# AIGC-Audio/AudioGPT

Hardware: AMD Instinct MI355X
Metric: generated audio-seconds/sec (10s clip, 100 DDIM steps) [3 independent batches of 8 prompts in flight per GPU] (higher is better)
Workload: dtype bf16x3; 1 GPU; Make-An-Audio T2A batch=8/GPU, 100 DDIM steps, CFG 1.5, UNet+VAE+HiFi-GAN(16k), fp32 storage, bf16x3-split MFMA (hi/lo, fp32 accumulate; meets the fp32 parity gates); prompts_per_gpu=8, ddim_steps=100, mel_frames=624, hipgraph=True, batches_in_flight=3, cfg_lanes=1, concurrency_hint=3, parallelism=prompt-sharded x1 (RCCL bcast cond / gather wav)

## Files before the change

### audiogpt_amd/_lib.py

```python
import ctypes as C
import os

import torch

_HERE = os.path.dirname(os.path.abspath(__file__))
LIB_PATH = os.environ.get("AUDIOGPT_AMD_LIB") or os.path.join(_HERE, "libaudiogpt_mi355x.so")


class MaaError(RuntimeError):
    pass


class maa_tensor(C.Structure):
    _fields_ = [("name", C.c_char_p), ("data", C.POINTER(C.c_float)), ("ndim", C.c_int), ("shape", C.c_int64 * 6)]


class maa_prof_row(C.Structure):
    _fields_ = [("name", C.c_char * 48), ("launches", C.c_int64), ("ms", C.c_double), ("flops", C.c_double),
                ("bytes", C.c_double)]


class maa_unet_config(C.Structure):
    _fields_ = [("in_channels", C.c_int), ("out_channels", C.c_int), ("model_channels", C.c_int),
                ("num_res_blocks", C.c_int),
# ... 114 lines not shown
    sig = {
        "maa_ctx_create": [ci, vp, C.POINTER(vp)],
        "maa_ctx_destroy": [vp],
        "maa_ctx_synchronize": [vp],
        "maa_ctx_set_stream": [vp, vp],
        "maa_ctx_workspace_bytes": [vp, C.POINTER(C.c_size_t)],
        "maa_ctx_set_precision": [vp, ci],
        "maa_ctx_set_cfg_split": [vp, ci],
        "maa_ctx_set_concurrency": [vp, ci],
        "maa_ctx_reload_tuning": [vp],
        "maa_prof_begin": [vp, ci],
        "maa_prof_end": [vp, C.POINTER(maa_prof_row), ci, C.POINTER(ci)],
        "maa_unet_create": [vp, C.POINTER(maa_unet_config), C.POINTER(maa_tensor), ci, C.POINTER(vp)],
        "maa_unet_destroy": [vp],
        "maa_unet_set_context": [vp, vp, vp, ci, ci],
        "maa_unet_forward": [vp, vp, vp, vp, ci, ci, ci, vp],
        "maa_ddim_update": [vp, vp, vp, vp, cf, vp, C.c_int64, vp, vp],
        "maa_ddim_sample": [vp, vp, C.POINTER(maa_ddim_args), vp],
        "maa_ddim_stochastic_encode": [vp, vp, ci, cf, vp, vp, fp, fp, ci, vp, ci, ci, ci, ci, vp],
        "maa_ddim_decode": [vp, vp, C.POINTER(maa_ddim_args), ci, vp],
        "maa_ldm_plms_sample": [vp, vp, C.POINTER(maa_ddim_args), vp],
        "maa_ddpm_sample": [vp, vp, C.POINTER(maa_ddpm_args), vp],
        "maa_ddpm_update": [vp, vp, vp, vp, fp, fp, fp, fp, fp, ci, vp, cf, ci, ci, ci, ci, ci, vp, vp],
        "maa_vae_create": [vp, C.POINTER(maa_vae_config), C.POINTER(maa_tensor), ci, C.POINTER(vp)],
        "maa_vae_destroy": [vp],
        "maa_vae_decode": [vp, vp, vp, ci, ci, ci, cf, vp],
        "maa_vae_decode_spec": [vp, vp, vp, ci, ci, ci, cf, vp],
        "maa_vae_encode_moments": [vp, vp, vp, ci, ci, ci, vp],
        "maa_vocoder_create": [vp, C.POINTER(maa_vocoder_config), C.POINTER(maa_tensor), ci, C.POINTER(vp)],
        "maa_vocoder_destroy": [vp],
        "maa_vocoder_forward": [vp, vp, vp, ci, ci, vp],
        "maa_vocoder_forward_f0": [vp, vp, vp, vp, vp, vp, ci, ci, vp],
        "maa_diffnet_create": [vp, C.POINTER(maa_diffnet_config), C.POINTER(maa_tensor), ci, C.POINTER(vp)],
        "maa_diffnet_destroy": [vp],
        "maa_diffnet_forward": [vp, vp, vp, vp, vp, ci, ci, vp],
        "maa_plms_sample": [vp, vp, C.POINTER(maa_plms_args), vp],
        "maa_ds_ddpm_sample": [vp, vp, C.POINTER(maa_ds_ddpm_args), vp],
        "maa_ds_ddpm_update": [vp, vp, vp, vp, fp, fp, fp, fp, fp, ci, ci, ci, ci, ci, vp],
        "maa_encoder_create": [vp, C.POINTER(maa_encoder_config), C.POINTER(maa_tensor), ci, C.POINTER(vp)],
        "maa_encoder_destroy": [vp],
        "maa_encoder_text": [vp, vp, vp, ci, ci, vp],
        "maa_encoder_image": [vp, vp, vp, ci, vp],
        "maa_encoder_text_cls": [vp, vp, vp, ci, ci, vp],
        "maa_clap_audio_create": [vp, C.POINTER(maa_clap_audio_config), C.POINTER(maa_tensor), ci, C.POINTER(vp)],
        "maa_clap_audio_destroy": [vp],
        "maa_clap_audio_embed": [vp, vp, vp, ci, ci, vp, vp],
        "maa_clap_similarity": [vp, vp, vp, ci, ci, ci, cf, vp],
        "maa_spectral_create": [vp, C.POINTER(maa_spectral_config), fp, fp, C.POINTER(vp)],
        "maa_spectral_destroy": [vp],
        "maa_spectral_forward": [vp, vp, vp, ci, ci, vp],
        "maa_resampler_create": [vp, ci, ci, ci, ci, fp, C.POINTER(vp)],
        "maa_resampler_destroy": [vp],
        "maa_resampler_forward": [vp, vp, vp, ci, ci, vp],
        "maa_op_linear": [vp, vp, ci, ci, fp, fp, ci, ci, vp],
        "maa_op_conv": [vp, vp, ci, ci, ci, ci, fp, fp, ci, ci, ci, ci, ci, ci, ci, cf, vp, ci, ci],
        "maa_op_groupnorm": [vp, vp, ci, ci, ci, fp, fp, cf, ci, vp],
        "maa_op_layernorm": [vp, vp, ci, ci, fp, fp, cf, vp],
        "maa_op_attention": [vp, vp, vp, vp, ci, ci, ci, ci, ci, cf, vp],
        "maa_op_attention_ex": [vp, vp, ci, ci, vp, ci, ci, vp, ci, ci, ci, ci, ci, ci, ci, cf, vp, ci, ci, ci],
        "maa_op_conv_transpose1d": [vp, vp, ci, ci, ci, fp, fp, ci, ci, ci, cf, vp],
        "maa_op_snake_aa": [vp, vp, ci, ci, ci, fp, fp, ci, vp],
        "maa_op_bench_conv": [vp, ci, ci, ci, ci, ci, ci, ci, ci, C.POINTER(C.c_float)],
        "maa_calib": [vp, ci, C.POINTER(C.c_double)],
        "maa_op_mrf_pair": [vp, vp, ci, ci, ci, fp, fp, ci, ci, cf, fp, fp, ci, ci, cf, cf, ci, vp],
        "maa_op_groupnorm_ex": [vp, vp, ci, ci, vp, ci, ci, ci, ci, ci, fp, fp, cf, ci, vp, ci, vp],
        "maa_op_layernorm_ex": [vp, vp, ci, ci, fp, fp, cf, vp, ci],
        "maa_op_split32": [vp, vp, ci, ci, cf, ci, vp],
        "maa_unet_forward_split": [vp, vp, vp, vp, vp, ci, ci, ci, ci, ci, ci, ci, fp, vp],
        "maa_op_unfold": [vp, vp, ci, ci, ci, ci, ci, ci, ci, ci, vp],
        "maa_op_fold": [vp, vp, fp, ci, ci, ci, ci, ci, ci, ci, ci, vp],
    }
    for name, argtypes in sig.items():
        fn = getattr(lib, name)
        fn.argtypes = argtypes
        fn.restype = ci
    _lib = lib
    return lib


def check(status):
    if status != 0:
        raise MaaError("libaudiogpt_mi355x: %s (status %d)" % (load().maa_last_error().decode(), status))


def host_f32(t):
    t = t.detach().to(device="cpu", dtype=torch.float32).contiguous()
    return t, C.cast(t.data_ptr(), C.POINTER(C.c_float))


def tensor_list(state_dict):
    items = list(state_dict.items())
    arr = (maa_tensor * len(items))()
    keep = []
    for i, (name, t) in enumerate(items):
        ht, ptr = host_f32(t)
        bname = name.encode()
        keep.append((ht, bname))
        arr[i].name = bname
        arr[i].data = ptr
        arr[i].ndim = ht.dim()
        for d, s in enumerate(ht.shape):
            arr[i].shape[d] = s
    return arr, len(items), keep


def dptr(t):
    assert t.is_cuda and t.dtype == torch.float32 and t.is_contiguous(), (t.device, t.dtype, t.is_contiguous())
    return C.c_void_p(t.data_ptr())
# ... 1 lines not shown
```

### audiogpt_amd/backend.py

```python
import ctypes as C
import threading
import weakref

import numpy as np
import torch

from . import _lib as L


def default_precision():
    import os
    p = os.environ.get("AUDIOGPT_AMD_PRECISION", "bf16x3")
    if p not in Context.PRECISIONS:
        raise ValueError("AUDIOGPT_AMD_PRECISION must be one of %s" % sorted(Context.PRECISIONS))
    return p


_contexts = weakref.WeakSet()


def reload_tuning():
    for c in list(_contexts):
        c.reload_tuning()

# ... 26 lines not shown

    def reload_tuning(self):
        if getattr(self, "h", None):
            with self.lock:
                L.check(self.lib.maa_ctx_reload_tuning(self.h))

    def set_precision(self, precision):
        L.check(self.lib.maa_ctx_set_precision(self.h, self.PRECISIONS[precision]))
        self.precision = precision

    def set_cfg_split(self, mode):
        L.check(self.lib.maa_ctx_set_cfg_split(self.h, -1 if mode is None else int(bool(mode))))

    def set_concurrency(self, n):
        L.check(self.lib.maa_ctx_set_concurrency(self.h, -1 if n is None else int(n)))

    def synchronize(self):
        L.check(self.lib.maa_ctx_synchronize(self.h))

    def workspace_bytes(self):
        n = C.c_size_t()
        L.check(self.lib.maa_ctx_workspace_bytes(self.h, C.byref(n)))
        return n.value

    def prof_begin(self, detail=False):
        L.check(self.lib.maa_prof_begin(self.h, int(detail)))

    def prof_end(self):
        rows = (L.maa_prof_row * 512)()
        n = C.c_int()
        L.check(self.lib.maa_prof_end(self.h, rows, 512, C.byref(n)))
        return {rows[i].name.decode(): dict(launches=int(rows[i].launches), ms=rows[i].ms, flops=rows[i].flops,
                                            bytes=rows[i].bytes) for i in range(n.value)}

    def calib(self):
        out = {}
        for kind, key in ((0, "mfma_bf16_tflops"), (1, "copy_gbs"), (2, "l2_read_gbs"), (3, "infinity_cache_read_gbs")):
            v = C.c_double()
            L.check(self.lib.maa_calib(self.h, kind, C.byref(v)))
            out[key] = v.value
        return out

    def close(self):
        if getattr(self, "h", None):
            self.lib.maa_ctx_destroy(self.h)
            self.h = None

    def __del__(self):
        try:
            self.close()
        except Exception:
            pass

    def op_linear(self, a, w, b=None, geglu=False):
        a = _f32(a, self.device)
        M, K = a.shape
        N = w.shape[0]
        wt, wp = L.host_f32(w)
        bt, bp = L.host_f32(b) if b is not None else (None, None)
        y = torch.empty(M, N // 2 if geglu else N, device=self.device)
        L.check(self.lib.maa_op_linear(self.h, L.dptr(a), M, K, wp, bp, N, int(geglu), L.dptr(y)))
        return y

    def op_conv(self, x, w, b=None, stride=1, pad=0, dil=1, up=False, leaky=0.0, out_hw=None):
        x = _f32(x, self.device)
        B, Cin, H, W = x.shape
        Cout, _, KH, KW = w.shape
        if out_hw is None:
            He, We = (2 * H, 2 * W) if up else (H, W)
            ph = pad if KH > 1 else 0
            Ho = (He + 2 * ph - dil * (KH - 1) - 1) // stride + 1
            Wo = (We + 2 * pad - dil * (KW - 1) - 1) // stride + 1
        else:
            Ho, Wo = out_hw
        wt, wp = L.host_f32(w)
        bt, bp = L.host_f32(b) if b is not None else (None, None)
        y = torch.empty(B, Cout, Ho, Wo, device=self.device)
        L.check(self.lib.maa_op_conv(self.h, L.dptr(x), B, Cin, H, W, wp, bp, Cout, KH, KW, stride, pad, dil,
                                     int(up), float(leaky), L.dptr(y), Ho, Wo))
        return y

    def op_groupnorm(self, x, gamma, beta, eps, silu=False):
        x = _f32(x, self.device)
        B, Cc = x.shape[:2]
        HW = int(np.prod(x.shape[2:]))
        gt, gp = L.host_f32(gamma)
        bt, bp = L.host_f32(beta)
        y = torch.empty_like(x)
        L.check(self.lib.maa_op_groupnorm(self.h, L.dptr(x), B, Cc, HW, gp, bp, float(eps), int(silu), L.dptr(y)))
        return y

    def op_layernorm(self, x, gamma, beta, eps=1e-5):
        x = _f32(x, self.device)
        rows, Cc = x.reshape(-1, x.shape[-1]).shape
        gt, gp = L.host_f32(gamma)
        bt, bp = L.host_f32(beta)
        y = torch.empty_like(x)
        L.check(self.lib.maa_op_layernorm(self.h, L.dptr(x), rows, Cc, gp, bp, float(eps), L.dptr(y)))
        return y

    def op_attention(self, q, k, v, heads, alpha):
        q, k, v = _f32(q, self.device), _f32(k, self.device), _f32(v, self.device)
        B, Nq, Cc = q.shape
        Nk = k.shape[1]
        y = torch.empty_like(q)
        L.check(self.lib.maa_op_attention(self.h, L.dptr(q), L.dptr(k), L.dptr(v), B, heads, Cc // heads, Nq, Nk,
                                          float(alpha), L.dptr(y)))
        return y

    def op_attention_ex(self, q, ldq, hsq, k, ldk, hsk, v, ldv, hsv, B, heads, dh, Nq, Nk, alpha, out, ldo,
                        out_split=0, causal=0):
        for t in (q, k, v, out):
            assert t.is_cuda and t.dtype == torch.float32, (t.device, t.dtype)
        L.check(self.lib.maa_op_attention_ex(self.h, C.c_void_p(q.data_ptr()), int(ldq), int(hsq),
                                             C.c_void_p(k.data_ptr()), int(ldk), int(hsk),
                                             C.c_void_p(v.data_ptr()), int(ldv), int(hsv), int(B), int(heads), int(dh),
                                             int(Nq), int(Nk), float(alpha), C.c_void_p(out.data_ptr()), int(ldo),
                                             int(out_split), int(causal)))
        return out

    def op_groupnorm_ex(self, x1, ld1, C1, x2, ld2, C2, B, HW, groups, gamma, beta, eps, silu, out, out_split=0, raw=None):
        for t in (x1, x2, out, raw):
            assert t is None or (t.is_cuda and t.dtype == torch.float32), (t.device, t.dtype)
        gt, gp = L.host_f32(gamma)
        bt, bp = L.host_f32(beta)
        assert gt.numel() == C1 + C2 and bt.numel() == C1 + C2
        ptr = lambda t: C.c_void_p(t.data_ptr()) if t is not None else None
        L.check(self.lib.maa_op_groupnorm_ex(self.h, ptr(x1), int(ld1), int(C1), ptr(x2), int(ld2), int(C2), int(B), int(HW),
                                             int(groups), gp, bp, float(eps), int(silu), ptr(out), int(out_split), ptr(raw)))
        return out

    def op_layernorm_ex(self, x, gamma, beta, eps=1e-5, out_split=0):
# ... 951 lines not shown
```

### audiogpt_amd/csrc/api.cpp

```cpp
#include "models.h"

#include <cstdint>
#include <cstring>
#include <memory>

namespace maa {
const char* last_error_cstr();
}

struct maa_ctx {
    maa::Ctx c;
    bool owns_stream = false;
};
struct maa_unet {
    std::unique_ptr<maa::UNet> m;
};
struct maa_vae {
    std::unique_ptr<maa::VAE> m;
};
struct maa_vocoder {
    std::unique_ptr<maa::Vocoder> m;
};
struct maa_diffnet {
    std::unique_ptr<maa::DiffNet> m;
// ... 556 lines not shown
}

int maa_spectral_create(maa_ctx* ctx, const maa_spectral_config* cfg, const float* h_basis, const float* h_melw,
                        maa_spectral** out) {
    return guarded([&] {
        bind(ctx);
        MAA_CHECK(cfg && h_basis && h_melw && out, "bad spectral arguments");
        MAA_CHECK(cfg->n_fft > 0 && cfg->n_fft % 4 == 0 && cfg->hop > 0 && cfg->hop % 4 == 0 && cfg->n_freq == cfg->n_fft / 2 + 1 &&
                      cfg->n_mels > 0 && (cfg->pad_mode == 0 || cfg->pad_mode == 1) && (cfg->power == 1 || cfg->power == 2) &&
                      (cfg->log_kind == 0 || cfg->log_kind == 1) && cfg->amin > 0.f && (cfg->out_layout == 0 || cfg->out_layout == 1),
                  "bad spectral config (n_fft and hop must be multiples of 4)");
        auto* s = new maa_spectral;
        s->m.reset(new maa::Spectral(*cfg, h_basis, h_melw));
        *out = s;
    });
}
int maa_spectral_destroy(maa_spectral* s) {
    return guarded([&] { delete s; });
}
int maa_spectral_forward(maa_ctx* ctx, maa_spectral* s, const float* d_wav, int B, int n, float* d_out) {
    return guarded([&] {
        bind(ctx);
        MAA_CHECK(s && d_wav && d_out && B > 0 && n > 0, "bad spectral_forward arguments");
        MAA_CHECK(s->m->config().pad_mode == 0 || n > s->m->config().n_fft / 2, "signal too short for reflect padding");
        s->m->forward(ctx->c, d_wav, B, n, d_out);
    });
}

int maa_resampler_create(maa_ctx* ctx, int orig, int neu, int width, int klen, const float* h_kernels, maa_resampler** out) {
    return guarded([&] {
        bind(ctx);
        MAA_CHECK(out && h_kernels && orig > 0 && neu > 0 && width > 0 && klen > 0, "bad resampler arguments");
        auto* r = new maa_resampler;
        r->m.reset(new maa::Resampler(orig, neu, width, klen, h_kernels));
        *out = r;
    });
}
int maa_resampler_destroy(maa_resampler* r) {
    return guarded([&] { delete r; });
}
int maa_resampler_forward(maa_ctx* ctx, maa_resampler* r, const float* d_wav, int B, int n, float* d_out) {
    return guarded([&] {
        bind(ctx);
        MAA_CHECK(r && d_wav && d_out && B > 0 && n > 0, "bad resampler_forward arguments");
        r->m->forward(ctx->c, d_wav, B, n, d_out);
    });
}

static bool op_presplit(const maa::Ctx& c, int channels, bool other_prologue) {
    return c.tune.op_presplit && c.dtype != 0 && channels % 32 == 0 && !other_prologue;
}

int maa_op_linear(maa_ctx* ctx, const float* d_a, int M, int K, const float* h_w, const float* h_bias, int N,
                  int geglu, float* d_y) {
    return guarded([&] {
        bind(ctx);
        MAA_CHECK(d_a && h_w && d_y && M > 0 && K > 0 && N > 0, "bad op_linear arguments");
        OneShot s;
        s.add("w", h_w, {N, K});
        if (h_bias) s.add("b", h_bias, {N});
        maa::WeightStore ws(ctx->c.dtype != 0);
        maa::Ctx& c = ctx->c;
        MAA_CHECK(!geglu || h_bias, "geglu needs a bias");
        maa::PackedW pw = geglu ? ws.pack_geglu(s.sd, "w", "b") : ws.pack_conv(s.sd, "w", h_bias ? "b" : "", 1, 1);
        const bool pre = op_presplit(c, K, false);
        maa::run_sized(c, [&] {
            const float* a = d_a;
            if (pre) {
                float* sp = c.ws.alloc_f((size_t)M * K);
                maa::launch_split32_pack(c, d_a, M, K, sp);
                a = sp;
            }
            maa::linear_into(c, a, K, M, K, pw, nullptr, 0, d_y, geglu ? N / 2 : N, geglu, 0, pre ? M : 0);
        });
        MAA_HIP(hipStreamSynchronize(c.stream));
    });
}

int maa_op_conv(maa_ctx* ctx, const float* d_x, int B, int Cin, int H, int W, const float* h_w, const float* h_bias,
                int Cout, int KH, int KW, int stride, int pad, int dil, int upsample2, float leaky_slope, float* d_y,
                int Ho, int Wo) {
    return guarded([&] {
        bind(ctx);
        MAA_CHECK(d_x && h_w && d_y, "bad op_conv arguments");
        OneShot s;
        s.add("w", h_w, {Cout, Cin, KH, KW});
        if (h_bias) s.add("b", h_bias, {Cout});
        maa::WeightStore ws(ctx->c.dtype != 0);
        maa::Ctx& c = ctx->c;
        maa::PackedW pw = ws.pack_conv(s.sd, "w", h_bias ? "b" : "", KH, KW);
        maa::PackedW pw4;
        if (upsample2 && KH == 3 && KW == 3 && stride == 1 && pad == 1 && dil == 1 && leaky_slope == 0.f)
            pw4 = ws.pack_conv_up2(s.sd, "w", h_bias ? "b" : "");
        maa::run_sized(c, [&] {
            maa::T4 x = maa::alloc_t(c, B, H, W, Cin);
            maa::launch_nchw_to_nhwc(c, d_x, B, Cin, H * W, x.p);
            if (!pw4.w && op_presplit(c, Cin, leaky_slope != 0.f)) {
                maa::T4 xs = maa::alloc_t(c, B, H, W, Cin);
                maa::launch_split32_pack(c, x.p, (long long)B * H * W, Cin, xs.p);
                xs.split = true;
                x = xs;
            }
            if (x.split && Cout <= 4 && h_bias && KH == 3 && KW == 3 && stride == 1 && pad == 1 && dil == 1 && !upsample2 && c.tune.up2) {
                maa::PackedW pn = ws.pack_narrow3x3(s.sd, "w", "b");
                if (maa::launch_narrow_conv3x3(c, x.p, Cin, B, H, W, Cin, pn.w, pn.bias, Cout, d_y)) return;
            }
            maa::T4 y = maa::alloc_t(c, B, Ho, Wo, Cout);
            maa::ConvOpt o;
            o.KH = KH;
            o.KW = KW;
            o.stride = stride;
            o.pad = pad;
            o.dil = dil;
            o.up = upsample2;
            if (leaky_slope != 0.f) {
                o.a_act = 1;
                o.a_slope = leaky_slope;
            }
            if (!(pw4.w && maa::conv_up2_into(c, x, pw4, y))) maa::conv_into(c, x, nullptr, pw, o, y);
            maa::launch_nhwc_to_nchw(c, y.p, B, Cout, Ho * Wo, d_y, Cout);
        });
        MAA_HIP(hipStreamSynchronize(c.stream));
    });
}

int maa_calib(maa_ctx* ctx, int kind, double* out_value) {
    return guarded([&] {
        bind(ctx);
        MAA_CHECK(out_value && kind >= 0 && kind <= 3, "bad calib arguments");
        *out_value = maa::calib_run(ctx->c, kind);
    });
}

int maa_op_groupnorm(maa_ctx* ctx, const float* d_x, int B, int C, int HW, const float* h_gamma, const float* h_beta,
                     float eps, int silu, float* d_y) {
    return guarded([&] {
        bind(ctx);
        MAA_CHECK(d_x && h_gamma && h_beta && d_y, "bad op_groupnorm arguments");
        maa::WeightStore ws(ctx->c.dtype != 0);
        maa::Ctx& c = ctx->c;
        float* g = ws.upload(std::vector<float>(h_gamma, h_gamma + C));
        float* b = ws.upload(std::vector<float>(h_beta, h_beta + C));
        maa::run_sized(c, [&] {
            maa::T4 x = maa::alloc_t(c, B, 1, HW, C), y = maa::alloc_t(c, B, 1, HW, C);
            maa::launch_nchw_to_nhwc(c, d_x, B, C, HW, x.p);
            maa::launch_groupnorm(c, x.p, C, C, nullptr, 0, 0, B, HW, 32, g, b, eps, silu, y.p);
            maa::launch_nhwc_to_nchw(c, y.p, B, C, HW, d_y, C);
        });
        MAA_HIP(hipStreamSynchronize(c.stream));
    });
}

int maa_op_layernorm(maa_ctx* ctx, const float* d_x, int rows, int C, const float* h_gamma, const float* h_beta,
                     float eps, float* d_y) {
    return guarded([&] {
        bind(ctx);
        MAA_CHECK(d_x && h_gamma && h_beta && d_y, "bad op_layernorm arguments");
        maa::WeightStore ws(ctx->c.dtype != 0);
        maa::Ctx& c = ctx->c;
        float* g = ws.upload(std::vector<float>(h_gamma, h_gamma + C));
        float* b = ws.upload(std::vector<float>(h_beta, h_beta + C));
        maa::launch_layernorm(c, d_x, rows, C, g, b, eps, d_y);
        MAA_HIP(hipStreamSynchronize(c.stream));
    });
}

int maa_op_attention(maa_ctx* ctx, const float* d_q, const float* d_k, const float* d_v, int B, int heads, int dh,
                     int Nq, int Nk, float alpha, float* d_y) {
    return guarded([&] {
        bind(ctx);
// ... 312 lines not shown
```

### audiogpt_amd/csrc/igemm_dma2.hip

```cpp
#include "igemm_epilogue.h"

#include <cstdio>
#include <cstdlib>
#include <cstring>
#include <type_traits>

namespace maa {

namespace {

template <int BM, int BN, int WGM, int WGN, int NS, int TERMS>
__global__ __launch_bounds__(64 * WGM * WGN) void igemm_dma2_kernel(const IGemm p, int ntiles, int tiles, int Nb,
                                                                     int cps, int items, float* __restrict__ part) {
    constexpr int NW = WGM * WGN, NTH = 64 * NW;
    constexpr int WTM = BM / WGM, WTN = BN / WGN;
    constexpr int MI = WTM / 32, NI = WTN / 32;
    constexpr int ROWS = BM + BN;
    constexpr int STAGE = ROWS * 128;
    constexpr int AI = BM / 8 / NW, BI = BN / 8 / NW;
    constexpr int IPW = AI + BI;
    static_assert(BM % (8 * NW) == 0 && BN % (8 * NW) == 0 && NW % 2 == 0, "copy assignment");
    static_assert(WTM % 32 == 0 && WTN % 32 == 0 && BM % 32 == 0, "tile");
    static_assert(NS >= 3 && (NS - 2) * IPW <= 63, "stages / vmcnt field");
    extern __shared__ __attribute__((aligned(1024))) char smem[];
// ... 187 lines not shown
        zero_acc();
        c_w += w_step;
        if (c_w >= w_cnt) return false;
        c_rem = item_chunks(c_w);
        return true;
    };

    setup_item(g_w);
    c_rem = item_chunks(c_w);
#pragma unroll
    for (int s = 0; s < NS - 1; ++s) issue(s);

    {
        wait_vmcnt<(NS - 2) * IPW>();
        __builtin_amdgcn_s_barrier();
        Frags f0, f1;
        read_frags(smem, 0, f0);
        int st = 0;
        for (;;) {
            const char* cur = smem + st * STAGE;
            const int st_next = st + 1 == NS ? 0 : st + 1;
            const int st_fill = st == 0 ? NS - 1 : st - 1;
            read_frags(cur, 1, f1);
            __builtin_amdgcn_sched_barrier(0);
            mma(f0);
            __builtin_amdgcn_sched_barrier(0);
            wait_vmcnt<(NS - 3) * IPW>();
            __builtin_amdgcn_s_barrier();
            read_frags(smem + st_next * STAGE, 0, f0);
            __builtin_amdgcn_sched_barrier(0);
            static_for<0, TERMS * MI * NI>([&](auto xc) {
                constexpr int x = decltype(xc)::value;
                constexpr int t = x / (MI * NI) + (3 - TERMS), i = (x % (MI * NI)) / NI, j = x % NI;
                if constexpr (t == 0)
                    acc[i][j] = __builtin_amdgcn_mfma_f32_32x32x16_bf16(f1.al[i], f1.bh[j], acc[i][j], 0, 0, 0);
                else if constexpr (t == 1)
                    acc[i][j] = __builtin_amdgcn_mfma_f32_32x32x16_bf16(f1.ah[i], f1.bl[j], acc[i][j], 0, 0, 0);
                else
                    acc[i][j] = __builtin_amdgcn_mfma_f32_32x32x16_bf16(f1.ah[i], f1.bh[j], acc[i][j], 0, 0, 0);
                if constexpr (x < IPW) copy1(st_fill, xc);
                __builtin_amdgcn_sched_barrier(0);
            });
            if constexpr (IPW > TERMS * MI * NI)
                static_for<TERMS * MI * NI, IPW>([&](auto jc) { copy1(st_fill, jc); });
            advance();
            st = st_next;
            if (--c_rem == 0)
                if (!finish_item()) break;
        }
    }
    wait_vmcnt<0>();
}

template <int JW>
__global__ void splitk_reduce_kernel(const IGemm p, const float* __restrict__ part, int S, int tiles, int ntiles, int Nb,
                                     int BM, int BN, int WGN, int MI, int NI) {
    const int NTH = blockDim.x;
    const int tid = threadIdx.x, lane = tid & 63, wid = tid >> 6;
    const int njb = NI / JW, nblk = MI * njb;
    const int wi = xcd_contiguous((int)blockIdx.x, (int)gridDim.x);
    const int tile = wi / nblk, blk = wi - tile * nblk;
    const int i = blk / njb, j = (blk - i * njb) * JW;
    const int mt = tile / ntiles, nt = tile - mt * ntiles;
    const int wm = wid / WGN, wn = wid - wm * WGN;
    const int WTM = 32 * MI, WTN = 32 * NI;
    f32x16 acc[1][JW];
    const long long slab = (long long)(MI * NI * 4) * NTH * 4;
#pragma unroll
    for (int jj = 0; jj < JW; ++jj) {
        const float* src = part + (long long)tile * slab + ((long long)((i * NI + j + jj) * 4) * NTH + tid) * 4;
        f32x4 v[4];
#pragma unroll
        for (int q = 0; q < 4; ++q) v[q] = *reinterpret_cast<const f32x4*>(src + (long long)q * NTH * 4);
        for (int s = 1; s < S; ++s) {
            const float* sp = src + (long long)s * tiles * slab;
#pragma unroll
            for (int q = 0; q < 4; ++q) v[q] += *reinterpret_cast<const f32x4*>(sp + (long long)q * NTH * 4);
        }
#pragma unroll
        for (int q = 0; q < 4; ++q)
#pragma unroll
            for (int e = 0; e < 4; ++e) acc[0][jj][4 * q + e] = v[q][e];
    }
    const int rpb = p.Hout * p.Wout;
    igemm_epilogue<1, JW>(p, acc, mt * BM + wm * WTM + i * 32, nt * BN + wn * WTN + j * 32, lane & 31, lane >> 5, 0, Nb, rpb);
}

template <int BM, int BN, int WGM, int WGN, int NS>
void launch_one(const Ctx& ctx, const IGemm& p, int Nb, int S, float* part) {
    constexpr int NW = WGM * WGN, NTH = 64 * NW;
    constexpr int MI = BM / WGM / 32, NI = BN / WGN / 32;
    const int ncols = p.N * (p.geglu ? 2 : 1);
    const int mtiles = (p.M + BM - 1) / BM, ntiles = (ncols + BN - 1) / BN;
    const int tiles = mtiles * ntiles;
    const int nchunks = p.K / BK;
    const int cps = (nchunks + S - 1) / S;
    const int Seff = (nchunks + cps - 1) / cps;
    MAA_CHECK(Seff == S, "split-K plan leaves an empty slice");
    MAA_CHECK(!p.geglu || NI % 2 == 0, "GEGLU needs value / gate block pairs inside a wave");
    constexpr size_t lds = (size_t)NS * (BM + BN) * 128;
    static_assert(lds <= 163840, "LDS per workgroup");
    const long long items = (long long)tiles * S;
    long long grid = items;
    {
        const int per_cu = (int)(163840 / lds) < 32 / NW ? (int)(163840 / lds) : 32 / NW;
        const long long cap = (long long)device_cu_count(ctx.device) * (per_cu < 1 ? 1 : per_cu);
        if (grid > cap) grid = cap;
    }
    auto go = [&](auto kern) {
        ensure_dynamic_lds(reinterpret_cast<const void*>(kern), ctx.device, (int)lds);
        hipLaunchKernelGGL(kern, dim3((unsigned)grid), dim3(NTH), lds, ctx.stream, p, ntiles, tiles, Nb, cps, (int)items,
                           S > 1 ? part : nullptr);
    };
    if (ctx.dtype == 2)
        go(igemm_dma2_kernel<BM, BN, WGM, WGN, NS, 1>);
    else
        go(igemm_dma2_kernel<BM, BN, WGM, WGN, NS, 3>);
    if (S > 1) launch_splitk_reduce(ctx, p, part, S, tiles, ntiles, Nb, BM, BN, WGN, MI, NI, NTH);
}

}

void launch_splitk_reduce(const Ctx& ctx, const IGemm& p, const float* part, int S, int tiles, int ntiles, int Nb, int BM,
                          int BN, int WGN, int MI, int NI, int NTH) {
    if (p.geglu && NI % 2 == 0) {
        hipLaunchKernelGGL(splitk_reduce_kernel<2>, dim3((unsigned)(tiles * MI * (NI / 2))), dim3(NTH), 0, ctx.stream, p, part, S,
                           tiles, ntiles, Nb, BM, BN, WGN, MI, NI);
        return;
    }
    MAA_CHECK(!p.geglu, "split-K reduce: GEGLU needs value / gate block pairs inside a wave");
    hipLaunchKernelGGL(splitk_reduce_kernel<1>, dim3((unsigned)(tiles * MI * NI)), dim3(NTH), 0, ctx.stream, p, part, S, tiles,
                       ntiles, Nb, BM, BN, WGN, MI, NI);
}

bool igemm_dma2_takes(const Ctx& ctx, const IGemm& p, IGemmPlan& pl) {
    const int ncols = p.N * (p.geglu ? 2 : 1);
    int S = 0;
    if (!ctx.tune.dma2.empty()) {
        if (ctx.tune.dma2 == "off") return false;
        int cfg = 0, ns = 4, pipe = 1, s = 1, kmin = 0, kmax = 1 << 30;
        const int k = std::sscanf(ctx.tune.dma2.c_str(), "%d,%d,%d,%d,%d,%d", &cfg, &ns, &pipe, &s, &kmin, &kmax);
        if (k >= 4) {
            if (p.K < kmin) return false;
            if (p.K <= kmax) S = s < 1 ? 1 : s;
        }
    }
    if (S == 0) {
        if (p.K < 2048 || ncols < 128 || p.geglu) return false;
        S = 2;
    }
    pl.engine = IGemmPlan::DMA2;
    pl.cfg = 0;
    pl.S = fit_slices(p.K / BK, S);
    return true;
}

void launch_igemm_dma2(const Ctx& ctx, const IGemm& p, const IGemmPlan& pl, float* part) {
    MAA_CHECK(pl.S == 1 || part != nullptr, "igemm_dma2: split-K needs its slab workspace");
    launch_one<128, 128, 2, 2, 4>(ctx, p, pl.Nb, pl.S, part);
}

}
```

### audiogpt_amd/csrc/igemm_epilogue.h

```cpp
#pragma once
#include "igemm_device.h"
#include "maa_internal.h"

namespace maa {

__device__ __forceinline__ float fast_erff(float x) {
    const float t = fminf(fabsf(x), 4.0f);
    const float s = t * t;
    float r = -5.654105860e-04f;
    r = fmaf(r, s, 4.923277665e-03f);
    r = fmaf(r, s, -2.671638510e-02f);
    r = fmaf(r, s, 1.128036441e-01f);
    r = fmaf(r, s, -3.761234978e-01f);
    r = fmaf(r, s, 1.128379127e+00f);
    const float small = r * t;
    float q = 1.330939039e-05f;
    q = fmaf(q, t, -3.175720346e-04f);
    q = fmaf(q, t, 3.436867598e-03f);
    q = fmaf(q, t, -2.262198592e-02f);
    q = fmaf(q, t, 1.033189800e-01f);
    q = fmaf(q, t, 6.390933195e-01f);
    q = fmaf(q, t, 1.125925949e+00f);
    q = fmaf(q, t, 7.569686250e-04f);
    const float large = 1.0f - __builtin_amdgcn_exp2f(q * -1.4426950408889634f);
    return copysignf(t < 1.0f ? small : large, x);
}

__device__ __forceinline__ void settle(float& x) { asm volatile("" : "+v"(x)); }

__device__ __forceinline__ void store_split_pair(float* row, int n, float v) {
    const __bf16 h = (__bf16)v;
    const unsigned hb = __builtin_bit_cast(unsigned short, h);
    const __bf16 l = (__bf16)(v - __builtin_bit_cast(float, hb << 16));
    const unsigned lb = __builtin_bit_cast(unsigned short, l);
    const bool even = (n & 1) == 0;
    const unsigned mine = even ? lb : hb;
    const unsigned theirs = (unsigned)__builtin_amdgcn_update_dpp(0, (int)mine, 0xB1, 0xF, 0xF, false);
    unsigned* o = reinterpret_cast<unsigned*>(reinterpret_cast<unsigned short*>(row) + (n >> 5) * 64 + ((n & 31) & ~1) + (even ? 0 : 32));
    *o = even ? (hb | (theirs << 16)) : (theirs | (lb << 16));
}

template <int MI, int NI, bool PAIR>
__device__ __forceinline__ void igemm_epilogue_impl(const IGemm& p, f32x16 (&acc)[MI][NI], int m_base, int n_base,
                                                    int lrow, int lk, long long coff, int Nb, int rpb) {
    float* cp = p.c + coff;
    const float* resp = p.res ? p.res + coff : nullptr;
    if (p.geglu) {
        if constexpr (NI % 2 == 0) {
#pragma unroll
            for (int i = 0; i < MI; ++i)
#pragma unroll
                for (int j = 0; j < NI; j += 2) {
                    const int cpk = n_base + j * 32 + lrow;
                    const int ncol = (cpk >> 6) * 32 + lrow;
                    if (cpk + 32 < Nb && ncol < p.N) {
                        float bv = p.bias ? p.bias[cpk] : 0.f;
                        float bg = p.bias ? p.bias[cpk + 32] : 0.f;
                        settle(bv);
                        settle(bg);
                        float outv[16];
#pragma unroll
                        for (int r = 0; r < 16; ++r) {
                            const float val = acc[i][j][r] * p.alpha + bv;
                            const float g = acc[i][j + 1][r] * p.alpha + bg;
                            const float gl = 0.5f * g * (1.f + fast_erff(g * 0.70710678118654752440f));
                            outv[r] = val * gl;
                        }
#pragma unroll
                        for (int r = 0; r < 16; ++r) {
                            const int m = m_base + i * 32 + (r & 3) + 8 * (r >> 2) + 4 * lk;
                            if (m < p.M) {
                                if (p.c_split)
                                    store_split_pair(cp + (long long)m * p.ldc, ncol, outv[r]);
                                else
                                    cp[(long long)m * p.ldc + ncol] = outv[r];
                            }
                        }
                    }
                }
        }
        return;
    }
#pragma unroll
    for (int i = 0; i < MI; ++i) {
        const int mb = m_base + i * 32;
        const int b0 = mb / rpb;
        const int nextb = (b0 + 1) * rpb;
#pragma unroll
        for (int j = 0; j < NI; ++j) {
            const int n = n_base + j * 32 + lrow;
            if (n < p.N) {
                float bias = p.bias ? p.bias[n] : 0.f;
                float ra[16], rs[16], cv[16];
                long long mc[16];
#pragma unroll
                for (int r = 0; r < 16; ++r) {
                    const int m = mb + (r & 3) + 8 * (r >> 2) + 4 * lk;
                    mc[r] = m < p.M ? m : p.M - 1;
                    ra[r] = rs[r] = cv[r] = 0.f;
                }
                if (p.rowadd) {
#pragma unroll
                    for (int r = 0; r < 16; ++r) {
                        const int bb = rpb >= 32 ? (mc[r] < nextb ? b0 : b0 + 1) : (int)(mc[r] / rpb);
                        ra[r] = p.rowadd[(long long)bb * p.ld_rowadd + n];
                    }
                }
                if (resp) {
#pragma unroll
                    for (int r = 0; r < 16; ++r) rs[r] = resp[mc[r] * p.ldr + n];
                }
                if (p.accumulate && !p.c_split) {
#pragma unroll
                    for (int r = 0; r < 16; ++r) cv[r] = cp[mc[r] * p.ldc + n];
                }
                settle(bias);
#pragma unroll
                for (int r = 0; r < 16; ++r) {
                    settle(ra[r]);
                    settle(rs[r]);
                    settle(cv[r]);
                }
                float outv[16];
#pragma unroll
                for (int r = 0; r < 16; ++r) {
                    float v = acc[i][j][r] * p.alpha + bias;
                    if (p.rowadd) v += ra[r];
                    if (resp) v += rs[r];
                    if (p.act == 1) v = tanhf(v);
                    else if (p.act == 2) v = fmaxf(v, 0.f);
                    else if (p.act == 3) v = 0.5f * v * (1.f + fast_erff(v * 0.70710678118654752440f));
                    else if (p.act == 4) v = v > 0.f ? v : v * p.act_slope;
                    v *= p.out_scale;
                    if (p.accumulate && !p.c_split) v += cv[r];
                    outv[r] = v;
                }
                if constexpr (PAIR) {
                    const bool even = (lrow & 1) == 0;
#pragma unroll
                    for (int rp = 0; rp < 8; ++rp) {
                        const float keep = even ? outv[2 * rp] : outv[2 * rp + 1];
                        const float give = even ? outv[2 * rp + 1] : outv[2 * rp];
                        const float got = __builtin_bit_cast(float, __builtin_amdgcn_update_dpp(0, __builtin_bit_cast(int, give), 0xB1, 0xF, 0xF, false));
                        const int r = 2 * rp + (even ? 0 : 1);
                        const int m = mb + (r & 3) + 8 * (r >> 2) + 4 * lk;
                        if (m < p.M) {
                            const f32x2 v2 = even ? f32x2{keep, got} : f32x2{got, keep};
                            *reinterpret_cast<f32x2*>(cp + (long long)m * p.ldc + (n & ~1)) = v2;
                        }
                    }
                } else {
#pragma unroll
                    for (int r = 0; r < 16; ++r) {
                        const int m = mb + (r & 3) + 8 * (r >> 2) + 4 * lk;
                        if (m < p.M) {
                            if (p.c_split)
                                store_split_pair(cp + (long long)m * p.ldc, n, outv[r]);
                            else
                                cp[(long long)m * p.ldc + n] = outv[r];
                            if (p.c2) {
                                const float w = outv[r] > 0.f ? outv[r] : outv[r] * p.c2_slope;
                                store_split_pair(p.c2 + coff + (long long)m * p.ldc2, n, w);
                            }
                        }
                    }
                }
            }
        }
    }
}

template <int MI, int NI>
__device__ __forceinline__ void igemm_epilogue(const IGemm& p, f32x16 (&acc)[MI][NI], int m_base, int n_base, int lrow,
                                               int lk, long long coff, int Nb, int rpb) {
    const bool pair = !p.geglu && !p.c_split && p.c2 == nullptr && (p.N & 1) == 0 && (p.ldc & 1) == 0 && (coff & 1) == 0 &&
                      (reinterpret_cast<uintptr_t>(p.c) & 7) == 0;
    if (pair)
        igemm_epilogue_impl<MI, NI, true>(p, acc, m_base, n_base, lrow, lk, coff, Nb, rpb);
    else
        igemm_epilogue_impl<MI, NI, false>(p, acc, m_base, n_base, lrow, lk, coff, Nb, rpb);
}

}
```

### include/maa.h

```cpp
#ifndef MAA_H_
#define MAA_H_

#include <stddef.h>
#include <stdint.h>

#ifdef __cplusplus
extern "C" {
#endif

typedef enum maa_status {
    MAA_OK = 0,
    MAA_ERR_INVALID = -1,
    MAA_ERR_HIP = -2,
    MAA_ERR_INTERNAL = -3
} maa_status;

typedef struct maa_ctx maa_ctx;
typedef struct maa_unet maa_unet;
typedef struct maa_vae maa_vae;
typedef struct maa_vocoder maa_vocoder;

const char* maa_last_error(void);
const char* maa_version(void);

// ... 164 lines not shown

typedef struct maa_encoder_config {
    int kind;
    int layers, width, heads, mlp_dim, d_proj;
    int vocab, max_positions;
    int patch, image;
    float ln_eps;
} maa_encoder_config;
typedef struct maa_encoder maa_encoder;
int maa_encoder_create(maa_ctx* ctx, const maa_encoder_config* cfg, const maa_tensor* tensors, int n_tensors,
                       maa_encoder** out);
int maa_encoder_destroy(maa_encoder* e);
int maa_encoder_text(maa_ctx* ctx, maa_encoder* e, const int* d_ids, int B, int L, float* d_out);
int maa_encoder_image(maa_ctx* ctx, maa_encoder* e, const float* d_img, int B, float* d_out);

int maa_encoder_text_cls(maa_ctx* ctx, maa_encoder* e, const int* d_ids, int B, int L, float* d_out);

typedef struct maa_clap_audio_config {
    int mel_bins, n_blocks, channels[8];
    int out_emb, d_proj;
    float bn_eps;
} maa_clap_audio_config;
typedef struct maa_clap_audio maa_clap_audio;
int maa_clap_audio_create(maa_ctx* ctx, const maa_clap_audio_config* cfg, const maa_tensor* tensors, int n_tensors,
                          maa_clap_audio** out);
int maa_clap_audio_destroy(maa_clap_audio* a);
int maa_clap_audio_embed(maa_ctx* ctx, maa_clap_audio* a, const float* d_logmel, int B, int T, float* d_embedding,
                         float* d_z);
int maa_clap_similarity(maa_ctx* ctx, const float* d_audio, const float* d_text, int Na, int Nt, int D, float scale,
                        float* d_out);

typedef struct maa_spectral_config {
    int n_fft, hop, n_freq, n_mels;
    int pad_mode;
    int power;
    int log_kind;
    float amin, ref;
    int out_layout;
} maa_spectral_config;
typedef struct maa_spectral maa_spectral;
int maa_spectral_create(maa_ctx* ctx, const maa_spectral_config* cfg, const float* h_basis, const float* h_melw,
                        maa_spectral** out);
int maa_spectral_destroy(maa_spectral* s);
int maa_spectral_forward(maa_ctx* ctx, maa_spectral* s, const float* d_wav, int B, int n, float* d_out);

typedef struct maa_resampler maa_resampler;
int maa_resampler_create(maa_ctx* ctx, int orig, int neu, int width, int klen, const float* h_kernels, maa_resampler** out);
int maa_resampler_destroy(maa_resampler* r);
int maa_resampler_forward(maa_ctx* ctx, maa_resampler* r, const float* d_wav, int B, int n, float* d_out);

int maa_calib(maa_ctx* ctx, int kind, double* out_value);

int maa_op_linear(maa_ctx* ctx, const float* d_a, int M, int K, const float* h_w, const float* h_bias, int N,
                  int geglu, float* d_y);
int maa_op_conv(maa_ctx* ctx, const float* d_x, int B, int Cin, int H, int W, const float* h_w, const float* h_bias,
                int Cout, int KH, int KW, int stride, int pad, int dil, int upsample2, float leaky_slope,
                float* d_y, int Ho, int Wo);
int maa_op_groupnorm(maa_ctx* ctx, const float* d_x, int B, int C, int HW, const float* h_gamma,
                     const float* h_beta, float eps, int silu, float* d_y);
int maa_op_layernorm(maa_ctx* ctx, const float* d_x, int rows, int C, const float* h_gamma, const float* h_beta,
                     float eps, float* d_y);
int maa_op_attention(maa_ctx* ctx, const float* d_q, const float* d_k, const float* d_v, int B, int heads, int dh,
                     int Nq, int Nk, float alpha, float* d_y);
int maa_op_attention_ex(maa_ctx* ctx, const float* d_q, int ldq, int hsq, const float* d_k, int ldk, int hsk,
                        const float* d_v, int ldv, int hsv, int B, int heads, int dh, int Nq, int Nk, float alpha,
                        float* d_y, int ldo, int out_split, int causal);
int maa_op_groupnorm_ex(maa_ctx* ctx, const float* d_x1, int ld1, int C1, const float* d_x2, int ld2, int C2, int B, int HW,
                        int groups, const float* h_gamma, const float* h_beta, float eps, int silu, float* d_y, int out_split,
                        float* d_raw);
int maa_op_layernorm_ex(maa_ctx* ctx, const float* d_x, int rows, int C, const float* h_gamma, const float* h_beta, float eps,
                        float* d_y, int out_split);
int maa_op_split32(maa_ctx* ctx, const float* d_x, int rows, int C, float slope, int unpack, float* d_y);
int maa_op_conv_transpose1d(maa_ctx* ctx, const float* d_x, int B, int Cin, int L, const float* h_w,
                            const float* h_bias, int Cout, int k, int stride, float leaky_slope, float* d_y);
int maa_op_bench_conv(maa_ctx* ctx, int B, int H, int W, int Cin, int Cout, int taps, int pre_split, int iters,
                      float* ms_per_launch);
int maa_op_snake_aa(maa_ctx* ctx, const float* d_x, int B, int C, int L, const float* h_alpha, const float* h_beta,
                    int logscale, float* d_y);
int maa_op_mrf_pair(maa_ctx* ctx, const float* d_x, int B, int C, int L, const float* h_w1, const float* h_b1, int k1, int d1,
                    float slope1, const float* h_w2, const float* h_b2, int k2, int d2, float slope2, float out_scale,
                    int accumulate, float* d_out);
int maa_op_unfold(maa_ctx* ctx, const float* d_x, int B, int C, int H, int W, int kh, int kw, int sh, int sw, float* d_out);
int maa_op_fold(maa_ctx* ctx, const float* d_crops, const float* h_weight, int B, int C, int H, int W, int kh, int kw, int sh, int sw,
                float* d_out);

#ifdef __cplusplus
}
#endif
#endif
```

Measured before the change: 134.6 audio-seconds/sec.

## Template split-K reduce geometry, specialize rowadd epilogue, extend op test entry points

Makes the split-K reduce kernel's tile and wave geometry compile-time template parameters with launch bounds, instantiating only the three geometries in use. The GEMM epilogue gains a template flag that loads the per-batch row-add from a base pointer plus a select when a 32-row block spans at most two batches, and it splits activation into its own pass. The single-op linear and conv test entry points gain residual, row-add and split32-output arguments. The kernel changes target register pressure and index arithmetic in the epilogue and reduce, at the cost of more template instances and a hard error for any geometry not instantiated.

```diff
diff --git a/audiogpt_amd/_lib.py b/audiogpt_amd/_lib.py
--- a/audiogpt_amd/_lib.py
+++ b/audiogpt_amd/_lib.py
@@ -190,8 +190,8 @@
         "maa_resampler_create": [vp, ci, ci, ci, ci, fp, C.POINTER(vp)],
         "maa_resampler_destroy": [vp],
         "maa_resampler_forward": [vp, vp, vp, ci, ci, vp],
-        "maa_op_linear": [vp, vp, ci, ci, fp, fp, ci, ci, vp],
-        "maa_op_conv": [vp, vp, ci, ci, ci, ci, fp, fp, ci, ci, ci, ci, ci, ci, ci, cf, vp, ci, ci],
+        "maa_op_linear": [vp, vp, ci, ci, fp, fp, ci, ci, vp, vp, ci],
+        "maa_op_conv": [vp, vp, ci, ci, ci, ci, fp, fp, ci, ci, ci, ci, ci, ci, ci, cf, vp, ci, ci, vp, vp, ci],
         "maa_op_groupnorm": [vp, vp, ci, ci, ci, fp, fp, cf, ci, vp],
         "maa_op_layernorm": [vp, vp, ci, ci, fp, fp, cf, vp],
         "maa_op_attention": [vp, vp, vp, vp, ci, ci, ci, ci, ci, cf, vp],
diff --git a/audiogpt_amd/backend.py b/audiogpt_amd/backend.py
--- a/audiogpt_amd/backend.py
+++ b/audiogpt_amd/backend.py
@@ -102,17 +102,21 @@
         except Exception:
             pass
 
-    def op_linear(self, a, w, b=None, geglu=False):
+    def op_linear(self, a, w, b=None, geglu=False, res=None, split_out=False):
         a = _f32(a, self.device)
         M, K = a.shape
         N = w.shape[0]
         wt, wp = L.host_f32(w)
         bt, bp = L.host_f32(b) if b is not None else (None, None)
         y = torch.empty(M, N // 2 if geglu else N, device=self.device)
-        L.check(self.lib.maa_op_linear(self.h, L.dptr(a), M, K, wp, bp, N, int(geglu), L.dptr(y)))
+        r = _f32(res, self.device) if res is not None else None
+        assert r is None or tuple(r.shape) == tuple(y.shape)
+        L.check(self.lib.maa_op_linear(self.h, L.dptr(a), M, K, wp, bp, N, int(geglu), L.dptr(y),
+                                       L.dptr(r) if r is not None else None, int(split_out)))
         return y
 
-    def op_conv(self, x, w, b=None, stride=1, pad=0, dil=1, up=False, leaky=0.0, out_hw=None):
+    def op_conv(self, x, w, b=None, stride=1, pad=0, dil=1, up=False, leaky=0.0, out_hw=None, rowadd=None, res=None,
+                split_out=False):
         x = _f32(x, self.device)
         B, Cin, H, W = x.shape
         Cout, _, KH, KW = w.shape
@@ -125,9 +129,14 @@
             Ho, Wo = out_hw
         wt, wp = L.host_f32(w)
         bt, bp = L.host_f32(b) if b is not None else (None, None)
-        y = torch.empty(B, Cout, Ho, Wo, device=self.device)
+        y = torch.empty((B, Ho, Wo, Cout) if split_out else (B, Cout, Ho, Wo), device=self.device)
+        ra = _f32(rowadd, self.device) if rowadd is not None else None
+        r = _f32(res, self.device) if res is not None else None
+        assert ra is None or tuple(ra.shape) == (B, Cout)
+        assert r is None or tuple(r.shape) == (B, Cout, Ho, Wo)
         L.check(self.lib.maa_op_conv(self.h, L.dptr(x), B, Cin, H, W, wp, bp, Cout, KH, KW, stride, pad, dil,
-                                     int(up), float(leaky), L.dptr(y), Ho, Wo))
+                                     int(up), float(leaky), L.dptr(y), Ho, Wo, L.dptr(ra) if ra is not None else None,
+                                     L.dptr(r) if r is not None else None, int(split_out)))
         return y
 
     def op_groupnorm(self, x, gamma, beta, eps, silu=False):
diff --git a/audiogpt_amd/csrc/api.cpp b/audiogpt_amd/csrc/api.cpp
--- a/audiogpt_amd/csrc/api.cpp
+++ b/audiogpt_amd/csrc/api.cpp
@@ -632,10 +632,12 @@
 }
 
 int maa_op_linear(maa_ctx* ctx, const float* d_a, int M, int K, const float* h_w, const float* h_bias, int N,
-                  int geglu, float* d_y) {
+                  int geglu, float* d_y, const float* d_res, int c_split) {
     return guarded([&] {
         bind(ctx);
         MAA_CHECK(d_a && h_w && d_y && M > 0 && K > 0 && N > 0, "bad op_linear arguments");
+        MAA_CHECK(!c_split || N % 32 == 0, "op_linear: split32 output needs a multiple of 32 columns");
+        MAA_CHECK(!geglu || (!d_res && !c_split), "op_linear: GEGLU takes neither a residual nor split32 output here");
         OneShot s;
         s.add("w", h_w, {N, K});
         if (h_bias) s.add("b", h_bias, {N});
@@ -651,7 +653,7 @@
                 maa::launch_split32_pack(c, d_a, M, K, sp);
                 a = sp;
             }
-            maa::linear_into(c, a, K, M, K, pw, nullptr, 0, d_y, geglu ? N / 2 : N, geglu, 0, pre ? M : 0);
+            maa::linear_into(c, a, K, M, K, pw, d_res, N, d_y, geglu ? N / 2 : N, geglu, 0, pre ? M : 0, c_split);
         });
         MAA_HIP(hipStreamSynchronize(c.stream));
     });
@@ -659,10 +661,13 @@
 
 int maa_op_conv(maa_ctx* ctx, const float* d_x, int B, int Cin, int H, int W, const float* h_w, const float* h_bias,
                 int Cout, int KH, int KW, int stride, int pad, int dil, int upsample2, float leaky_slope, float* d_y,
-                int Ho, int Wo) {
+                int Ho, int Wo, const float* d_rowadd, const float* d_res, int c_split) {
     return guarded([&] {
         bind(ctx);
         MAA_CHECK(d_x && h_w && d_y, "bad op_conv arguments");
+        const bool extras = d_rowadd || d_res || c_split;
+        MAA_CHECK(!extras || !upsample2, "op_conv: row add, residual and split32 output are not combined with the upsample");
+        MAA_CHECK(!c_split || Cout % 32 == 0, "op_conv: split32 output needs a multiple of 32 channels");
         OneShot s;
         s.add("w", h_w, {Cout, Cin, KH, KW});
         if (h_bias) s.add("b", h_bias, {Cout});
@@ -681,7 +686,7 @@
                 xs.split = true;
                 x = xs;
             }
-            if (x.split && Cout <= 4 && h_bias && KH == 3 && KW == 3 && stride == 1 && pad == 1 && dil == 1 && !upsample2 && c.tune.up2) {
+            if (x.split && Cout <= 4 && h_bias && KH == 3 && KW == 3 && stride == 1 && pad == 1 && dil == 1 && !upsample2 && !extras && c.tune.up2) {
                 maa::PackedW pn = ws.pack_narrow3x3(s.sd, "w", "b");
                 if (maa::launch_narrow_conv3x3(c, x.p, Cin, B, H, W, Cin, pn.w, pn.bias, Cout, d_y)) return;
             }
@@ -696,6 +701,19 @@
             if (leaky_slope != 0.f) {
                 o.a_act = 1;
                 o.a_slope = leaky_slope;
+            }
+            o.rowadd = d_rowadd;
+            o.ld_rowadd = Cout;
+            if (d_res) {
+                maa::T4 r = maa::alloc_t(c, B, Ho, Wo, Cout);
+                maa::launch_nchw_to_nhwc(c, d_res, B, Cout, Ho * Wo, r.p);
+                o.res = r.p;
+            }
+            if (c_split) {
+                o.c_split = 1;
+                y.p = d_y;
+                maa::conv_into(c, x, nullptr, pw, o, y);
+                return;
             }
             if (!(pw4.w && maa::conv_up2_into(c, x, pw4, y))) maa::conv_into(c, x, nullptr, pw, o, y);
             maa::launch_nhwc_to_nchw(c, y.p, B, Cout, Ho * Wo, d_y, Cout);
diff --git a/audiogpt_amd/csrc/igemm_dma2.hip b/audiogpt_amd/csrc/igemm_dma2.hip
--- a/audiogpt_amd/csrc/igemm_dma2.hip
+++ b/audiogpt_amd/csrc/igemm_dma2.hip
@@ -263,20 +263,20 @@
     wait_vmcnt<0>();
 }
 
-template <int JW>
-__global__ void splitk_reduce_kernel(const IGemm p, const float* __restrict__ part, int S, int tiles, int ntiles, int Nb,
-                                     int BM, int BN, int WGN, int MI, int NI) {
-    const int NTH = blockDim.x;
+template <int JW, int MI, int NI, int WGN, int NTH>
+__global__ __launch_bounds__(NTH) void splitk_reduce_kernel(const IGemm p, const float* __restrict__ part, int S, int tiles,
+                                                           int ntiles, int Nb) {
+    constexpr int njb = NI / JW, nblk = MI * njb;
+    constexpr int WTM = 32 * MI, WTN = 32 * NI;
+    constexpr int BM = WTM * (NTH / 64 / WGN), BN = WTN * WGN;
+    constexpr long long slab = (long long)(MI * NI * 4) * NTH * 4;
     const int tid = threadIdx.x, lane = tid & 63, wid = tid >> 6;
-    const int njb = NI / JW, nblk = MI * njb;
     const int wi = xcd_contiguous((int)blockIdx.x, (int)gridDim.x);
     const int tile = wi / nblk, blk = wi - tile * nblk;
     const int i = blk / njb, j = (blk - i * njb) * JW;
     const int mt = tile / ntiles, nt = tile - mt * ntiles;
     const int wm = wid / WGN, wn = wid - wm * WGN;
-    const int WTM = 32 * MI, WTN = 32 * NI;
     f32x16 acc[1][JW];
-    const long long slab = (long long)(MI * NI * 4) * NTH * 4;
 #pragma unroll
     for (int jj = 0; jj < JW; ++jj) {
         const float* src = part + (long long)tile * slab + ((long long)((i * NI + j + jj) * 4) * NTH + tid) * 4;
@@ -295,6 +295,21 @@
     }
     const int rpb = p.Hout * p.Wout;
     igemm_epilogue<1, JW>(p, acc, mt * BM + wm * WTM + i * 32, nt * BN + wn * WTN + j * 32, lane & 31, lane >> 5, 0, Nb, rpb);
+}
+
+template <int MI, int NI, int WGN, int NTH>
+void launch_reduce_geom(const Ctx& ctx, const IGemm& p, const float* part, int S, int tiles, int ntiles, int Nb) {
+    auto go = [&](auto kern, int blocks) {
+        hipLaunchKernelGGL(kern, dim3((unsigned)blocks), dim3(NTH), 0, ctx.stream, p, part, S, tiles, ntiles, Nb);
+    };
+    if (p.geglu) {
+        if constexpr (NI % 2 == 0)
+            go(splitk_reduce_kernel<2, MI, NI, WGN, NTH>, tiles * MI * (NI / 2));
+        else
+            MAA_CHECK(false, "split-K reduce: GEGLU needs value / gate block pairs inside a wave");
+        return;
+    }
+    go(splitk_reduce_kernel<1, MI, NI, WGN, NTH>, tiles * MI * NI);
 }
 
 template <int BM, int BN, int WGM, int WGN, int NS>
@@ -334,14 +349,15 @@
 
 void launch_splitk_reduce(const Ctx& ctx, const IGemm& p, const float* part, int S, int tiles, int ntiles, int Nb, int BM,
                           int BN, int WGN, int MI, int NI, int NTH) {
-    if (p.geglu && NI % 2 == 0) {
-        hipLaunchKernelGGL(splitk_reduce_kernel<2>, dim3((unsigned)(tiles * MI * (NI / 2))), dim3(NTH), 0, ctx.stream, p, part, S,
-                           tiles, ntiles, Nb, BM, BN, WGN, MI, NI);
-        return;
-    }
-    MAA_CHECK(!p.geglu, "split-K reduce: GEGLU needs value / gate block pairs inside a wave");
-    hipLaunchKernelGGL(splitk_reduce_kernel<1>, dim3((unsigned)(tiles * MI * NI)), dim3(NTH), 0, ctx.stream, p, part, S, tiles,
-                       ntiles, Nb, BM, BN, WGN, MI, NI);
+    MAA_CHECK(BM == 32 * MI * (NTH / 64 / WGN) && BN == 32 * NI * WGN, "split-K reduce: tile and wave geometry disagree");
+    if (MI == 1 && NI == 5 && WGN == 1 && NTH == 512)
+        launch_reduce_geom<1, 5, 1, 512>(ctx, p, part, S, tiles, ntiles, Nb);
+    else if (MI == 2 && NI == 2 && WGN == 2 && NTH == 512)
+        launch_reduce_geom<2, 2, 2, 512>(ctx, p, part, S, tiles, ntiles, Nb);
+    else if (MI == 2 && NI == 2 && WGN == 2 && NTH == 256)
+        launch_reduce_geom<2, 2, 2, 256>(ctx, p, part, S, tiles, ntiles, Nb);
+    else
+        MAA_CHECK(false, "split-K reduce: no instantiation for this workgroup geometry");
 }
 
 bool igemm_dma2_takes(const Ctx& ctx, const IGemm& p, IGemmPlan& pl) {
diff --git a/audiogpt_amd/csrc/igemm_epilogue.h b/audiogpt_amd/csrc/igemm_epilogue.h
--- a/audiogpt_amd/csrc/igemm_epilogue.h
+++ b/audiogpt_amd/csrc/igemm_epilogue.h
@@ -40,7 +40,7 @@
     *o = even ? (hb | (theirs << 16)) : (theirs | (lb << 16));
 }
 
-template <int MI, int NI, bool PAIR>
+template <int MI, int NI, bool PAIR, bool RSEL>
 __device__ __forceinline__ void igemm_epilogue_impl(const IGemm& p, f32x16 (&acc)[MI][NI], int m_base, int n_base,
                                                     int lrow, int lk, long long coff, int Nb, int rpb) {
     float* cp = p.c + coff;
@@ -84,7 +84,7 @@
 #pragma unroll
     for (int i = 0; i < MI; ++i) {
         const int mb = m_base + i * 32;
-        const int b0 = mb / rpb;
+        const int b0 = (mb < p.M ? mb : p.M - 1) / rpb;
         const int nextb = (b0 + 1) * rpb;
 #pragma unroll
         for (int j = 0; j < NI; ++j) {
@@ -100,10 +100,13 @@
                     ra[r] = rs[r] = cv[r] = 0.f;
                 }
                 if (p.rowadd) {
-#pragma unroll
-                    for (int r = 0; r < 16; ++r) {
-                        const int bb = rpb >= 32 ? (mc[r] < nextb ? b0 : b0 + 1) : (int)(mc[r] / rpb);
-                        ra[r] = p.rowadd[(long long)bb * p.ld_rowadd + n];
+                    if constexpr (RSEL) {
+                        const float* ra0 = p.rowadd + (long long)b0 * p.ld_rowadd + n;
+#pragma unroll
+                        for (int r = 0; r < 16; ++r) ra[r] = ra0[mc[r] < nextb ? 0 : p.ld_rowadd];
+                    } else {
+#pragma unroll
+                        for (int r = 0; r < 16; ++r) ra[r] = p.rowadd[(long long)((int)mc[r] / rpb) * p.ld_rowadd + n];
                     }
                 }
                 if (resp) {
@@ -127,11 +130,22 @@
                     float v = acc[i][j][r] * p.alpha + bias;
                     if (p.rowadd) v += ra[r];
                     if (resp) v += rs[r];
-                    if (p.act == 1) v = tanhf(v);
-                    else if (p.act == 2) v = fmaxf(v, 0.f);
-                    else if (p.act == 3) v = 0.5f * v * (1.f + fast_erff(v * 0.70710678118654752440f));
-                    else if (p.act == 4) v = v > 0.f ? v : v * p.act_slope;
-                    v *= p.out_scale;
+                    outv[r] = v;
+                }
+                if (p.act != 0) {
+#pragma unroll
+                    for (int r = 0; r < 16; ++r) {
+                        float v = outv[r];
+                        if (p.act == 1) v = tanhf(v);
+                        else if (p.act == 2) v = fmaxf(v, 0.f);
+                        else if (p.act == 3) v = 0.5f * v * (1.f + fast_erff(v * 0.70710678118654752440f));
+                        else if (p.act == 4) v = v > 0.f ? v : v * p.act_slope;
+                        outv[r] = v;
+                    }
+                }
+#pragma unroll
+                for (int r = 0; r < 16; ++r) {
+                    float v = outv[r] * p.out_scale;
                     if (p.accumulate && !p.c_split) v += cv[r];
                     outv[r] = v;
                 }
@@ -175,10 +189,15 @@
                                                int lk, long long coff, int Nb, int rpb) {
     const bool pair = !p.geglu && !p.c_split && p.c2 == nullptr && (p.N & 1) == 0 && (p.ldc & 1) == 0 && (coff & 1) == 0 &&
                       (reinterpret_cast<uintptr_t>(p.c) & 7) == 0;
-    if (pair)
-        igemm_epilogue_impl<MI, NI, true>(p, acc, m_base, n_base, lrow, lk, coff, Nb, rpb);
+    const bool rsel = !(p.rowadd && rpb < 32);
+    if (pair && rsel)
+        igemm_epilogue_impl<MI, NI, true, true>(p, acc, m_base, n_base, lrow, lk, coff, Nb, rpb);
+    else if (pair)
+        igemm_epilogue_impl<MI, NI, true, false>(p, acc, m_base, n_base, lrow, lk, coff, Nb, rpb);
+    else if (rsel)
+        igemm_epilogue_impl<MI, NI, false, true>(p, acc, m_base, n_base, lrow, lk, coff, Nb, rpb);
     else
-        igemm_epilogue_impl<MI, NI, false>(p, acc, m_base, n_base, lrow, lk, coff, Nb, rpb);
-}
-
-}
+        igemm_epilogue_impl<MI, NI, false, false>(p, acc, m_base, n_base, lrow, lk, coff, Nb, rpb);
+}
+
+}
diff --git a/include/maa.h b/include/maa.h
--- a/include/maa.h
+++ b/include/maa.h
@@ -240,10 +240,10 @@
 int maa_calib(maa_ctx* ctx, int kind, double* out_value);
 
 int maa_op_linear(maa_ctx* ctx, const float* d_a, int M, int K, const float* h_w, const float* h_bias, int N,
-                  int geglu, float* d_y);
+                  int geglu, float* d_y, const float* d_res, int c_split);
 int maa_op_conv(maa_ctx* ctx, const float* d_x, int B, int Cin, int H, int W, const float* h_w, const float* h_bias,
                 int Cout, int KH, int KW, int stride, int pad, int dil, int upsample2, float leaky_slope,
-                float* d_y, int Ho, int Wo);
+                float* d_y, int Ho, int Wo, const float* d_rowadd, const float* d_res, int c_split);
 int maa_op_groupnorm(maa_ctx* ctx, const float* d_x, int B, int C, int HW, const float* h_gamma,
                      const float* h_beta, float eps, int silu, float* d_y);
 int maa_op_layernorm(maa_ctx* ctx, const float* d_x, int rows, int C, const float* h_gamma, const float* h_beta,
```

Result: faster. 138.2 audio-seconds/sec (median of 6 runs) (+2.7%).
